# moss-lab/ScanFold

Hardware: NVIDIA B200
Metric: windows/sec (MFE+100 shuffles+ED) (higher is better)
Workload: dtype int32

## Files before the change

include/scanfold_b200.h:

```cpp
#ifndef SCANFOLD_B200_H
#define SCANFOLD_B200_H
#include <stdint.h>
#ifdef __cplusplus
extern "C" {
#endif
#if defined(__GNUC__)
#pragma GCC visibility push(default)
#endif

#define SFB_VERSION 100
#define SFB_INF 10000000

#define SFB_E_ARG (-1)
#define SFB_E_PARAMS (-2)
#define SFB_E_CUDA (-3)
#define SFB_E_STATE (-4)
#define SFB_E_RANGE (-5)

#define SFB_SHUFFLE_MONO 0
#define SFB_SHUFFLE_DI 1

typedef struct sfb_model {
    double temperature;
    int32_t max_bp_span;
// ... 69 lines not shown
int sfb_accumulate_export(sfb_partner_table *table, int row0, int n_rows, int32_t *d_count, int32_t *d_first_seen,
                          int64_t *d_sums);
int sfb_accumulate_merge(sfb_partner_table *table, int row0, int n_rows, const int32_t *d_count,
                         const int32_t *d_first_seen, const int64_t *d_sums);
int sfb_accumulate_compact(sfb_partner_table *table, int row0, int n_rows, int64_t *n_entries);
int sfb_accumulate_fetch(sfb_partner_table *table, int32_t *nparts, int32_t *partner, int32_t *count,
                         int32_t *first_seen, int64_t *sums);
int sfb_accumulate_launches(const sfb_partner_table *table);
void sfb_accumulate_free(sfb_partner_table *table);

typedef struct sfb_pairprob_table sfb_pairprob_table;
int sfb_pairprob_begin(int32_t L, int32_t W, int32_t step, int32_t first_window, int32_t n_windows,
                       sfb_pairprob_table **table);
int sfb_scan_plan_pairprob(sfb_scan_plan *plan, sfb_pairprob_table *table);
int sfb_pairprob_export(sfb_pairprob_table *table, int row0, int n_rows, int64_t *d_rows);
int sfb_pairprob_merge(sfb_pairprob_table *table, int row0, int n_rows, const int64_t *d_rows);
int sfb_pairprob_compact(sfb_pairprob_table *table, int row0, int n_rows, double cutoff, int64_t *n_pairs);
int sfb_pairprob_fetch(sfb_pairprob_table *table, double *paired, int32_t *i, int32_t *j, double *p);
void sfb_pairprob_free(sfb_pairprob_table *table);

#define SFB_MICROBENCH_ADDMIN 0
#define SFB_MICROBENCH_SMEM_LD32 1
#define SFB_MICROBENCH_DFMA 2
int sfb_microbench(int which, double *ops_per_s);

#if defined(__GNUC__)
#pragma GCC visibility pop
#endif
#ifdef __cplusplus
}
#endif
#endif
```

scanfold_b200/csrc/mfe3.cu:

```cuda
#include <cstddef>
#include <cstdio>
#include <cstdlib>
#include <type_traits>

#include "device_common.cuh"

namespace sfb {
namespace {

constexpr int INF16 = 16000;
constexpr int TABLE_ENV16 = 2000;
constexpr int FIN16 = 4000;
constexpr int LOW16 = -12000;
constexpr int R32 = 32;
constexpr int R16 = 16;
constexpr int SEG = 25;

struct alignas(16) Tab3 {
    short stack[64], mmI[200], mm1n[200], mm23[200], mmH[200];
    short mlclose[200];
    short mlstem[8 * 36];
    short ext[8 * 36];
    short tAU[8];
    short bulge1;
// ... 14 lines not shown
bool g_mfe3_ok = false;

constexpr int BIG = 1 << 20;


__device__ __forceinline__ int lds_s16(unsigned a) {
    int v;
    asm volatile("ld.shared.s16 %0, [%1];" : "=r"(v) : "r"(a));
    return v;
}
__device__ __forceinline__ unsigned lds_u32(unsigned a) {
    unsigned v;
    asm volatile("ld.shared.u32 %0, [%1];" : "=r"(v) : "r"(a));
    return v;
}
__device__ __forceinline__ int4 lds_v4(unsigned a) {
    int4 v;
    asm volatile("ld.shared.v4.s32 {%0, %1, %2, %3}, [%4];" : "=r"(v.x), "=r"(v.y), "=r"(v.z), "=r"(v.w) : "r"(a));
    return v;
}
__device__ __forceinline__ void sts_u16(unsigned a, int v) {
    asm volatile("st.shared.u16 [%0], %1;" ::"r"(a), "h"((short)v));
}

template <int P, bool FMG = false>
struct Smem3 {
    static constexpr int KSM = FMG ? 4 : 2;
    static constexpr int PR = P <= 64 ? P + 2 : ((P + 2 + 63) / 64) * 64 - 2;
    static constexpr int PRW = (P + 3) | 1;
    Tab3 tb;
    short ne[R32 * PR], no[R32 * PR], m8[R32 * PR];
    unsigned rpa[R32 * PRW];
    unsigned rpq[R32 * PRW];
    short g[R16 * PR];
    short rc[R16 * PR];
    short fm[FMG ? 8 : P * P];
    short decp[KSM * 8 * PR];
    short partc[4 * PR], parts[4 * PR];
    short f5[P + 8];
    static constexpr int LP = P;
    alignas(16) int list[(4 * LP + 16) * 4];
    unsigned char ctx[R16 * PR];
    unsigned char sx[P + 8];
    unsigned char sx5[P + 8], sx3[P + 8];
    alignas(16) int cnt[4];
    int wq[2];
    short scp[P + 8];
    int minv[32];
    int fbest[32];
    alignas(8) int stepinfo[(P / 2 + 4) * 2];
};

__host__ __device__ __forceinline__ int tri4(int d, int W) {
    return (d - 4) * W - ((d - 1) * d / 2 - 6);
}

__host__ __device__ __forceinline__ int ksplit(int D, int W, bool fmg = false) {
    if (fmg) return D >= 71 ? 4 : (D >= 36 ? 2 : 1);
    return (D < 36 || (W - 1 - D) / 2 + 1 <= 16) ? 1 : 2;
}

__device__ int hairpin_special3(const MfeTables *T, const Tab3 &tb, const unsigned char *sx, int i, int j, int type) {
    const int u = j - i - 1;
    int e = T->hairpin_len[u];
    auto key = [&](int n) {
        int k = 0, mul = 1;
        for (int t = 0; t < n; t++) {
            k += sx[i + 1 + t] * mul;
            mul *= 5;
        }
        return k;
    };
    if (u == 4) {
// ... 20 lines not shown
    if (nl == 0) return T->stack[type][t2];
    if (ns == 0) {
        int e = T->bulge[nl];
        if (nl == 1)
            e += T->stack[type][t2];
        else
            e += (type > 2 ? au : 0) + (t2 > 2 ? au : 0);
        return e;
    }
    if (ns == 1) {
        if (nl == 1) return T->int11[type][t2][si1][sj1];
        if (nl == 2) return n1 == 1 ? T->int21[type][t2][si1][sq1][sj1] : T->int21[t2][type][sq1][si1][sp1];
        return T->internal_loop[nl + 1] + min(T->max_ninio, (nl - ns) * T->ninio) + T->mismatch1nI[type][si1][sj1] +
               T->mismatch1nI[t2][sq1][sp1];
    }
    if (ns == 2) {
        if (nl == 2) return T->int22[type][t2][si1][sp1][sq1][sj1];
        if (nl == 3) return T->internal_loop[5] + T->ninio + T->mismatch23I[type][si1][sj1] + T->mismatch23I[t2][sq1][sp1];
    }
    return T->internal_loop[nl + ns] + min(T->max_ninio, (nl - ns) * T->ninio) + T->mismatchI[type][si1][sj1] +
           T->mismatchI[t2][sq1][sp1];
}

template <int P, bool FMG, class SMT>
__device__ bool traceback3(SMT &sm, const short *fm, const MfeTables *T, const short *cx, short *pt, int W, int lane) {
    const Tab3 &tb = sm.tb;
    const unsigned char *sx = sm.sx;
    const unsigned full = 0xffffffffu;
    static_assert(sizeof(sm.list) >= 3 * (P + 8) * sizeof(int), "the traceback stack lives in the list area");
    int *stk = reinterpret_cast<int *>(sm.list);
    auto ptype = [&](int a, int b) { return (int)tb.ptype[sx[a + 1] * 6 + sx[b + 1]]; };
    auto CC = [&](int i, int j) {
        const int v = cx[tri4(j - i, W) + i];
        return v >= FIN16 ? INF : v - tb.ext[ptype(i, j) * 36 + sx[i] * 6 + sx[j + 2]];
    };
    auto MM = [&](int i, int j) {
        if (j - i <= TURN) return INF;
        int v;
        if constexpr (FMG) v = __ldcg(fm + i * P + j);
        else v = fm[i * P + j];
        return v >= FIN16 ? INF : v;
    };
    for (int k = lane; k < W; k += 32) pt[k] = 0;
    int sp = 1;
    if (lane == 0) {
        stk[0] = 0;
        stk[1] = W - 1;
        stk[2] = 0;
    }
    __syncwarp();
    while (sp > 0) {
        sp--;
        int i = stk[3 * sp], j = stk[3 * sp + 1];
        const int ml = stk[3 * sp + 2];
        __syncwarp();
        bool have_pair = false;
        if (j < i + TURN + 1) continue;
        const int fij = ml ? MM(i, j) : (int)sm.f5[j + 1];
        const int mij1 = MM(i, j - 1);
        const int fi = ml ? (mij1 < INF ? mij1 + tb.MLbase : INF) : (int)sm.f5[j];
        auto push = [&](int a, int b, int c) {
            if (lane == 0) {
// ... 87 lines not shown
            if (traced) continue;
            const int en = cij - tb.mlclose[(tb.rtype[type] * 5 + sx[j]) * 5 + sx[i + 2]];
            int kf = -1;
            for (int k0 = i + 2 + TURN; k0 < j - 2 - TURN && kf < 0; k0 += 32) {
                const int k = k0 + lane;
                bool hit = false;
                if (k < j - 2 - TURN) {
                    const int a = MM(i + 1, k), b = MM(k + 1, j - 1);
                    hit = a < INF && b < INF && en == a + b;
                }
                const unsigned m = __ballot_sync(full, hit);
                if (m) kf = k0 + __ffs(m) - 1;
            }
            if (kf < 0) return false;
            push(i + 1, kf, 1);
            push(kf + 1, j - 1, 1);
            break;
        }
        __syncwarp();
    }
    return true;
}

template <int P, int NW, int OCC, bool FMG>
__global__ void __launch_bounds__(NW * 32, OCC)
mfe3_kernel(MfeLaunch L, const MfeTables *__restrict__ T, const Tab3 *__restrict__ gtab) {
    extern __shared__ __align__(16) unsigned char smem_raw[];
    using SM = Smem3<P, FMG>;
    SM &sm = *reinterpret_cast<SM *>(smem_raw);
    constexpr int NT = NW * 32, PR = SM::PR;
    const int tid = threadIdx.x, warp = tid >> 5, lane = tid & 31;
    const unsigned full = 0xffffffffu;
    {
        const int *src = reinterpret_cast<const int *>(gtab);
        int *dst = reinterpret_cast<int *>(&sm.tb);
        static_assert(sizeof(Tab3) % 4 == 0, "Tab3 is copied as 32-bit words");
        for (int k = tid; k < (int)(sizeof(Tab3) / 4); k += NT) dst[k] = src[k];
    }
    const Tab3 &tb = sm.tb;
    const unsigned char *sx = sm.sx;
    const int W = L.W;
    constexpr int LP = SM::LP;
    const int npairs = (W - TURN) / 2 + 1;
    for (int st = tid; st < npairs; st += NT) {
        const int d0 = TURN + 2 + 2 * st;
        const int nseg0 = d0 < W ? (W - d0 + SEG - 1) / SEG : 0, nseg1 = d0 + 1 < W ? (W - d0 - 1 + SEG - 1) / SEG : 0;
        const int nF = d0 - 2 < W ? (W - (d0 - 2) + 30) / 31 : 0;
        const int D = d0 + 1;
        const int ntile = D <= W - 1 ? (W - 1 - D) / 2 + 1 : 0;
        const int KS = ksplit(D, W, FMG), ksh = KS == 4 ? 2 : KS >> 1 ;
        const int kwsh = ntile > 16 ? 0 : (ntile > 8 ? 1 : 2), TPW = 32 >> kwsh;
        const int nT = ((ntile + TPW - 1) >> (5 - kwsh)) << ksh;
        reinterpret_cast<int2 *>(sm.stepinfo)[st] =
            make_int2(nseg0 | ((nseg0 + nseg1) << 8) | (nF << 16), ntile | (ksh << 8) | (kwsh << 12) | (nT << 16));
    }
    short *gC = reinterpret_cast<short *>(L.gscratch) + (size_t)blockIdx.x * L.gscratch_per_cta;
    auto ldfm = [&](const short *q) -> short {
        if constexpr (FMG) return __ldcg(q);
        else return *q;
    };
// ... 18 lines not shown
    const int UC = U < 12 ? U + 12 : (U > MAXLOOP ? MAXLOOP : U);
    const int UB10 = U < 11 ? 11 : (U > MAXLOOP ? MAXLOOP : U), UB18 = U < 20 ? 20 : (U > MAXLOOP ? MAXLOOP : U);
    const int UB26 = U < 28 ? 28 : (U > MAXLOOP ? MAXLOOP : U);
    const int kA = ((UA & 1) ? O_NO : O_NE) + 3 + (UA >> 1), kC = O_M8 + UC - 1;
    const int g6a = c3_sG6[0], g6b = c3_sG6[1], g6c = c3_sG6[2], g9 = c3_cap[9], g10 = c3_cap[10];

    auto build_list = [&](int d) {
        const int ncells = W - d, slot = d & 3;
        constexpr int NCH = (P + 31) / 32;
        int tt[NCH];
#pragma unroll
        for (int k = 0; k < NCH; k++) {
            const int i = k * 32 + lane;
            tt[k] = i < ncells ? tb.ptype[sm.sx5[i + 1] * 6 + sm.sx3[i + d + 1]] : 0;
        }
        int nl = 0;
#pragma unroll
        for (int k = 0; k < NCH; k++) {
            if (k * 32 < ncells) {
                const int i = k * 32 + lane, t = tt[k];
                const unsigned m = __ballot_sync(full, t != 0);
                if (t) {
                    const int mi = (t * 5 + sx[i + 2]) * 5 + sx[i + d];
                    const int4 en = make_int4(i, tb.mmI[mi], tb.mm1n[mi], tb.tAU[t]);
                    reinterpret_cast<int4 *>(sm.list)[slot * LP + nl + __popc(m & ((1u << lane) - 1))] = en;
                }
                nl += __popc(m);
            }
        }
        if (lane == 0) sm.cnt[slot] = nl;
    };
    auto decof = [&](int d, int xi) {
        if (d < 2 * TURN + 3) return INF16;
        const int Dsrc = (d & 1) ? ((xi & 1) ? d + 1 : d - 1) : d;
        const int ks = ksplit(Dsrc, W, FMG);
        int v = sm.decp[(d & 7) * PR + xi];
        for (int kp = 1; kp < ks; kp++) v = min(v, (int)sm.decp[(kp * 8 + (d & 7)) * PR + xi]);
        return v;
    };
    auto unit_P = [&](int d, int c) {
        const int slot = d & 3, n = sm.cnt[slot];
        const int idx = c * 32 + lane;
        const bool active = idx < n;
        const int i = active ? sm.list[(slot * LP + idx) * 4] : 0;
        const int j = i + d;
        const int type = tb.ptype[sx[i + 1] * 6 + sx[j + 1]];
        const int si1 = sx[i + 2], sj1 = sx[j];
        const int mi = (type * 5 + si1) * 5 + sj1;
        int aT = INF16;
        auto inner = [&](int u1, int u2, int &cc, int &t2, int &sp1, int &sq1) {
            const int dd = d - 2 - u1 - u2, p = i + 1 + u1, q = j - 1 - u2;
            const bool ok = dd > TURN;
            cc = ok ? sm.rc[(dd & (R16 - 1)) * PR + p] : INF16;
            t2 = ok ? sm.ctx[(dd & (R16 - 1)) * PR + p] : 0;
            sp1 = sx[p];
            sq1 = sx[q + 2];
        };
        int cc, t2, sp1, sq1;
        {
            inner(1, 1, cc, t2, sp1, sq1);
            aT = min(aT, cc + __ldg(&T->int11[type][t2][si1][sj1]));
            int eh = __ldg(&T->hairpin_len[d - 1]) + tb.mmH[mi];
            if (d <= 7 && active) eh = hairpin_special3(T, tb, sx, i, j, type);
            aT = min(aT, eh);
            inner(1, 2, cc, t2, sp1, sq1);
            aT = min(aT, cc + __ldg(&T->int21[type][t2][si1][sq1][sj1]));
            inner(2, 1, cc, t2, sp1, sq1);
            aT = min(aT, cc + __ldg(&T->int21[t2][type][sq1][si1][sp1]));
            inner(2, 2, cc, t2, sp1, sq1);
            aT = min(aT, cc + __ldg(&T->int22[type][t2][si1][sp1][sq1][sj1]));
            inner(2, 3, cc, t2, sp1, sq1);
            aT = min(aT, cc + tb.il5_ninio + tb.mm23[mi] + tb.mm23[(t2 * 5 + sq1) * 5 + sp1]);
            inner(3, 2, cc, t2, sp1, sq1);
            aT = min(aT, cc + tb.il5_ninio + tb.mm23[mi] + tb.mm23[(t2 * 5 + sq1) * 5 + sp1]);
            auto grow = [&](int dd, int p) { return dd > TURN ? (int)sm.g[(dd & (R16 - 1)) * PR + p] : INF16; };
            int aG = min(grow(d - 8, i + 3) + g6a, min(grow(d - 8, i + 4) + g6b, grow(d - 8, i + 5) + g6c));
            aG = min(aG, min(grow(d - 11, i + 3), grow(d - 11, i + 8)) + g9);
            aG = min(aG, min(grow(d - 12, i + 3), grow(d - 12, i + 9)) + g10);
            aT = min(aT, aG + tb.mmI[mi]);
        }
        if (active) sm.parts[slot * PR + i] = (short)min(aT, INF16);
    };

    int minv = 0;

    auto unit_S = [&](int d, int sg) {
        const int ncells = W - d;
        const int x = sg * SEG - 7 + lane;
        const bool valid = x >= 0 && x < ncells;
        const int i = valid ? x : 0, j = i + d;
        const int c5 = sm.sx5[i + 1], c3 = sm.sx3[j + 1];
        const int pc = sm.partc[(d & 3) * PR + i], ps = sm.parts[(d & 3) * PR + i];
        const int o2 = ((d - 2) & (R16 - 1)) * PR + i + 1, o3 = ((d - 3) & (R16 - 1)) * PR + i + 1;
        const int rc2 = sm.rc[o2], cx2 = sm.ctx[o2];
        const int rc3a = sm.rc[o3], cx3a = sm.ctx[o3], rc3b = sm.rc[o3 + 1], cx3b = sm.ctx[o3 + 1];
        const int dm = decof(d - 2, i + 1);
        const int si0 = sx[i], si2 = sx[i + 2], sj0 = sx[j], sj2 = sx[j + 2];
        int scs = 0;
        if (L.sc) scs = sm.scp[i] + sm.scp[j - 1];
        const int t = valid ? tb.ptype[c5 * 6 + c3] : 0;
        const int t2 = tb.rtype[t];
        const int st2 = tb.stack[t * 8 + cx2], st3a = tb.stack[t * 8 + cx3a], st3b = tb.stack[t * 8 + cx3b];
        const int mlc = tb.mlclose[(t2 * 5 + sj0) * 5 + si2];
        const int m2 = (t2 * 5 + sj2) * 5 + si0;
        const int xI = tb.mmI[m2], x1n = tb.mm1n[m2], xAU = tb.tAU[t2];
        int e = min(pc, ps);
        if (d - 2 > TURN) e = min(e, rc2 + st2 + scs);
        if (d - 3 > TURN) e = min(e, min(rc3a + st3a, rc3b + st3b) + tb.bulge1);
        e = min(e, dm + mlc);
        if (!t || e >= FIN16) e = INF16;
        int vg = INF16, v1 = INF16, vb = INF16;
        if (t && i > 0 && j < W - 1 && e < FIN16) {
            vg = e + xI;
            v1 = e + x1n;
            vb = e + xAU;
        }
        const int g1 = __shfl_up_sync(full, vg, 1), g2 = __shfl_up_sync(full, vg, 2);
        const int g3 = __shfl_up_sync(full, vg, 3), g4 = __shfl_up_sync(full, vg, 4);
        const int ne = min(g2, min(min(g1, g3) + tb.w2, min(vg, g4) + tb.w4));
        const int no = min(min(g1, g2) + tb.w1, min(vg, g3) + tb.w3);
        int m8 = min(vg, g1);
        m8 = min(m8, __shfl_up_sync(full, m8, 2));
        m8 = min(m8, __shfl_up_sync(full, m8, 4));
        if (valid && lane >= 7) {
            minv = min(minv, e);
            const int o16 = (d & (R16 - 1)) * PR + i, o32 = (d & (R32 - 1)) * PR + i;
            sm.rc[o16] = (short)e;
            sm.ctx[o16] = (unsigned char)t2;
            sm.g[o16] = (short)vg;
            {
                short *wa = reinterpret_cast<short *>(sm.rpa) + 2 * ((d & (R32 - 1)) * PRW + i);
                short *wq = reinterpret_cast<short *>(sm.rpq) + 2 * ((d & (R32 - 1)) * PRW + j);
                wa[0] = (short)vb;
                if (i > 0) wa[-1] = (short)v1;
                wq[0] = (short)vb;
                wq[3] = (short)v1;
            }
            sm.ne[o32] = (short)ne;
            sm.no[o32] = (short)no;
            sm.m8[o32] = (short)m8;
            gC[tri4(d, W) + i] = (short)(e < FIN16 ? e + tb.ext[t * 36 + sx[i] * 6 + sx[j + 2]] : INF16);
        }
    };

    auto unit_F = [&](int dA, int u) {
        const int nc0 = dA > TURN ? W - dA : 0, nc1 = dA + 1 < W ? W - dA - 1 : 0;
        const int x = u * 31 + lane;
        const bool v0 = x < nc0;
        const int xx = v0 ? x : max(nc0 - 1, 0);
        auto stemof = [&](int d, int xi) {
            const int o16 = (d & (R16 - 1)) * PR + xi;
            const int e = sm.rc[o16];
            const int t = tb.rtype[sm.ctx[o16]];
            return e < FIN16 ? e + tb.mlstem[t * 36 + sx[xi] * 6 + sx[xi + d + 2]] : INF16;
        };
        const int x1c = min(x, max(nc1 - 1, 0));
        const int s0 = min(decof(dA, xx), stemof(dA, xx));
        const int s1 = min(decof(dA + 1, x1c), stemof(dA + 1, x1c));
        int m0 = INF16;
        if (nc0 > 0) {
            m0 = s0;
            if (dA - 1 > TURN)
                m0 = min(m0, min((int)ldfm(fm + (xx + 1) * P + xx + dA), (int)ldfm(fm + xx * P + xx + dA - 1)) + tb.MLbase);
            if (m0 >= FIN16) m0 = INF16;
            if (v0) {
                minv = min(minv, m0);
                fm[x * P + x + dA] = (short)m0;
                fm[(x + dA) * P + x] = (short)m0;
            }
        }
        const int m0n = __shfl_down_sync(full, m0, 1);
        if (lane < 31 && x < nc1) {
            const int d = dA + 1;
            int m1 = min(s1, min(m0, m0n) + tb.MLbase);
// ... 61 lines not shown
                const unsigned a = pa[0], b = pb[0];
                acc0 = __viaddmin_s16x2(a, __byte_perm(b, 0, 0x1010), acc0);
                acc1 = __viaddmin_s16x2(a, __byte_perm(b, 0, 0x3232), acc1);
            }
        }
        if (kwsh >= 1) {
            acc0 = __vmins2(acc0, __shfl_xor_sync(full, acc0, 16));
            acc1 = __vmins2(acc1, __shfl_xor_sync(full, acc1, 16));
        }
        if (kwsh == 2) {
            acc0 = __vmins2(acc0, __shfl_xor_sync(full, acc0, 8));
            acc1 = __vmins2(acc1, __shfl_xor_sync(full, acc1, 8));
        }
        if (valid && kq == 0) {
            auto fin = [](int v) { return (short)(v >= FIN16 ? INF16 : v); };
            short *dp = sm.decp + kp * 8 * PR;
            dp[(D & 7) * PR + i] = fin((short)(acc0 & 0xffffu));
            dp[((D - 1) & 7) * PR + i + 1] = fin((int)acc0 >> 16);
            if (j + 1 < W) {
                dp[((D + 1) & 7) * PR + i] = fin((short)(acc1 & 0xffffu));
                dp[(D & 7) * PR + i + 1] = fin((int)acc1 >> 16);
            }
        }
    };

    for (int fold = blockIdx.x; fold < L.n_fold; fold += gridDim.x) {
        __syncthreads();
        for (int k = tid; k < W + 2; k += NT) {
            const bool edge = k == 0 || k == W + 1;
            const int code = edge ? 5 : L.seqs[(size_t)fold * W + k - 1];
            const char ch = (L.hc && !edge) ? (char)L.hc[(size_t)fold * W + k - 1] : '.';
            sm.sx[k] = (unsigned char)code;
            sm.sx5[k] = (unsigned char)((ch == 'x' || ch == '>') ? 5 : code);
            sm.sx3[k] = (unsigned char)((ch == 'x' || ch == '<') ? 5 : code);
        }
        {
            const int4 inf4 = make_int4(INF16 * 65537, INF16 * 65537, INF16 * 65537, INF16 * 65537);
            int4 *p = reinterpret_cast<int4 *>(sm.ne);
            constexpr int n16 = (int)((offsetof(SM, decp) - offsetof(SM, ne) + 15) / 16);
            for (int k = tid; k < n16; k += NT) p[k] = inf4;
            for (int k = tid; k < 4 * PR; k += NT) sm.partc[k] = INF16;
            if constexpr (FMG) {
                int4 *q = reinterpret_cast<int4 *>(fm);
                for (int k = tid; k < P * P / 8; k += NT) q[k] = inf4;
            }
        }
// ... 88 lines not shown
                int my = draw();
                while (my < total) {
                    const int nx = draw();
                    if (my < uP) {
                        unit_T(d0 + 1, my, ntile, ksh, kwsh);
                    } else if (my < uS) {
                        const int it = my - uP;
                        unit_P(it < nch2 ? d0 + 2 : d0 + 3, it < nch2 ? it : it - nch2);
                    } else if (my < uL) {
                        const int u = my - uS;
                        unit_S(u >= nseg0 ? d0 + 1 : d0, u >= nseg0 ? u - nseg0 : u);
                    } else if (my < uF) {
                        build_list(d0 + 4 + (my - uL));
                    } else if (my < uC) {
                        unit_F(d0 - 2, my - uF);
                    } else {
                        const int ci = my - uC, ds = ci >= nc2;
                        const int c = (ds ? ci - nc2 : ci) * CH;
                        unit_C(d0 + 2 + ds, c, min(c + CH, ds ? n3 : n2));
                    }
                    my = nx;
                }
            } else {
                const int uP = nS, uT = uP + nP, uF = uT + nT, uL = uF + nF, nH = uL + 2;
                for (int u = warp; u < nH; u += NW) {
                    if (u < uP) {
                        unit_S(u >= nseg0 ? d0 + 1 : d0, u >= nseg0 ? u - nseg0 : u);
                    } else if (u < uT) {
                        const int it = u - uP;
                        unit_P(it < nch2 ? d0 + 2 : d0 + 3, it < nch2 ? it : it - nch2);
                    } else if (u < uF) {
                        unit_T(d0 + 1, u - uT, ntile, ksh, kwsh);
                    } else if (u < uL) {
                        unit_F(d0 - 2, u - uF);
                    } else {
                        build_list(d0 + 4 + (u - uL));
                    }
                }
                int c = warp - nH % NW;
                if (c < 0) c += NW;
#pragma unroll 1
                for (int ds = 0; ds < 2; ds++) {
                    const int d = d0 + 2 + ds, n = ds ? n3 : n2;
                    if (c < n) {
                        const int slot = (d - 2 - UB) & (R32 - 1);
                        const unsigned sb = (unsigned)__cvta_generic_to_shared(smb);
                        const unsigned aA = sb + 2 * (kA + ((d - 2 - UA) & (R32 - 1)) * PR);
                        const unsigned aB10 = sb + 2 * (O_M8 + 10 + ((d - 2 - UB10) & (R32 - 1)) * PR);
                        const unsigned aB18 = sb + 2 * (O_M8 + 18 + ((d - 2 - UB18) & (R32 - 1)) * PR);
                        const unsigned aB26 = sb + 2 * (O_M8 + 26 + ((d - 2 - UB26) & (R32 - 1)) * PR);
                        const unsigned aC = sb + 2 * (kC + ((d - 2 - UC) & (R32 - 1)) * PR);
                        const unsigned aR = (unsigned)__cvta_generic_to_shared(sm.rpa + slot * PRW + 1);
                        const unsigned aL = (unsigned)__cvta_generic_to_shared(sm.rpq + slot * PRW + d - 1);
                        const unsigned aP = (unsigned)__cvta_generic_to_shared(sm.partc + (d & 3) * PR);
                        unsigned aLst = (unsigned)__cvta_generic_to_shared(reinterpret_cast<const int4 *>(sm.list) + (d & 3) * LP + c);
                        int4 en = lds_v4(aLst);
                        for (; c < n; c += NW) {
                            const int i = en.x, eI = en.y, e1 = en.z, eB = en.w;
                            aLst += NW * 16;
                            en = lds_v4(aLst);
                            const unsigned i2 = 2 * i, i4 = 4 * i;
                            const unsigned wr = lds_u32(aR + i4), wl = lds_u32(aL + i4);
                            const int xa = lds_s16(aA + i2), xb10 = lds_s16(aB10 + i2), xb18 = lds_s16(aB18 + i2);
                            const int xb26 = lds_s16(aB26 + i2), xc = lds_s16(aC + i2);
                            const unsigned wm = __vmins2(wr, wl);
                            const int xb = (int)(short)(wm & 0xffffu), x1 = (int)wm >> 16;
                            int g = xa + cA;
                            g = __viaddmin_s32(xb10, cB10, g);
                            int g2 = xb18 + cB18;
                            g2 = __viaddmin_s32(xb26, cB26, g2);
                            g = __viaddmin_s32(xc, cC, g);
                            const int aB = xb + cSB, a1 = x1 + cS1;
                            int v = min(g, g2) + eI;
                            v = __viaddmin_s32(a1, e1, v);
                            v = __viaddmin_s32(aB, eB, v);
                            v = __reduce_min_sync(full, v);
                            if (lane == 0) sts_u16(aP + i2, v);
                        }
                    }
                    c -= n;
                }
            }
            __syncthreads();
        }

        {
            short *cx = sm.ne;
            const int ntri = tri4(W, W);
            for (int k = tid; k < ntri; k += NT) cx[k] = __ldcg(gC + k);
            for (int k = tid; k <= min(W, TURN + 1); k += NT) sm.f5[k] = 0;
            const int minw = __reduce_min_sync(full, minv);
            if (lane == 0) sm.minv[warp] = minw;
            __syncthreads();
            constexpr int LPR = 8, NPART = NW > LPR ? NW / LPR : 1;
            for (int len0 = TURN + 2; len0 <= W; len0 += LPR) {
                for (int t = warp % LPR; t < LPR; t += NW) {
                    const int len = len0 + t, j = len - 1, part = warp / LPR;
                    int best = INF16;
                    if (len <= W && part < NPART)
                        for (int i = lane + 32 * part; i <= min(j - TURN - 1, len0 - 1); i += 32 * NPART)
                            best = min(best, sm.f5[i] + cx[tri4(j - i, W) + i]);
                    best = __reduce_min_sync(full, best);
                    if (lane == 0 && part < NPART) sm.fbest[t + LPR * part] = best;
                }
                __syncthreads();
                if (tid == 0) {
// ... 2 lines not shown
#pragma unroll
                    for (int t = 0; t < LPR; t++) {
                        if (len0 + t <= W) {
#pragma unroll
                            for (int h = 0; h < NPART; h++) run = min(run, sm.fbest[t + LPR * h]);
#pragma unroll
                            for (int q = 0; q + 5 <= t; q++) {
                                const int i = len0 + q, j = len0 + t - 1;
                                run = min(run, f[q] + cx[tri4(j - i, W) + i]);
                            }
                            f[t] = run;
                            sm.f5[len0 + t] = (short)run;
                        }
                    }
                }
                __syncthreads();
            }
            int mv = sm.minv[0];
            for (int q = 1; q < NW; q++) mv = min(mv, sm.minv[q]);
            if (tid == 0) L.e_out[fold] = mv < LOW16 ? MFE_REDO : (int)sm.f5[W];
            if (L.pair_tbl && mv >= LOW16) {
                short *pt = sm.partc;
                if (warp == 0) {
                    const bool ok = traceback3<P, FMG>(sm, fm, T, cx, pt, W, lane);
                    if (!ok && lane == 0) L.e_out[fold] = MFE_REDO;
                }
                __syncthreads();
                for (int k = tid; k < W; k += NT) L.pair_tbl[(size_t)fold * W + k] = pt[k];
            }
        }
    }
}

template <int P, int NW, int OCC, bool FMG = false>
void launch_mfe3_t(const MfeLaunch &L, const MfeTables *d_tab, int n_sm, cudaStream_t stream) {
    const size_t smem = sizeof(Smem3<P, FMG>);
    static bool cfg = false;
    if (!cfg) {
        cudaFuncSetAttribute(mfe3_kernel<P, NW, OCC, FMG>, cudaFuncAttributeMaxDynamicSharedMemorySize, (int)smem);
        cfg = true;
    }
    const int grid = L.n_fold < n_sm * OCC ? L.n_fold : n_sm * OCC;
    mfe3_kernel<P, NW, OCC, FMG><<<grid, NW * 32, smem, stream>>>(L, d_tab, g_dtab3);
}

}

static_assert(sizeof(Smem3<200>) <= 227 * 1024, "the 200-nt configuration must fit one SM");
static_assert(sizeof(Smem3<300, true>) <= 227 * 1024, "the 300-nt configuration must fit one SM");
static_assert(300 * 300 % 8 == 0, "the global matrix is cleared with 16-byte stores");
bool mfe3_supports(int W) { return g_mfe3_ok && W >= 16 && W <= 300; }

size_t mfe3_scratch_shorts_per_cta(int W) {
    const size_t tri = ((size_t)tri4(W, W) + 63) & ~(size_t)63;
    return tri + (W > 200 ? (size_t)300 * 300 : 0);
}

int mfe3_max_ctas(int n_sm, int W) { return n_sm * (W <= 64 ? 4 : (W <= 120 ? 2 : 1)); }

void mfe3_upload_tables(const MfeTables &M) {
    static Tab3 h;
    bool fit = true;
    auto s16 = [&fit](int v) {
        fit = fit && v >= -TABLE_ENV16 && v <= TABLE_ENV16;
        return (short)v;
    };
    auto mm = [](int t, int a, int b) { return (t * 5 + a) * 5 + b; };
    static const int rt[8] = {0, 2, 1, 4, 3, 6, 5, 7};
    for (int a = 0; a < 8; a++)
        for (int b = 0; b < 8; b++) h.stack[a * 8 + b] = s16(M.stack[a][b]);
    for (int t = 0; t < 8; t++) {
        h.tAU[t] = s16(t > 2 ? M.TerminalAU : 0);
        h.rtype[t] = (unsigned char)rt[t];
        for (int a = 0; a < 5; a++)
            for (int b = 0; b < 5; b++) {
                h.mmI[mm(t, a, b)] = s16(M.mismatchI[t][a][b]);
                h.mm1n[mm(t, a, b)] = s16(M.mismatch1nI[t][a][b]);
                h.mm23[mm(t, a, b)] = s16(M.mismatch23I[t][a][b]);
                h.mmH[mm(t, a, b)] = s16(M.mismatchH[t][a][b]);
                h.mlclose[mm(t, a, b)] = s16(M.mismatchM[t][a][b] + (t > 2 ? M.TerminalAU : 0) + M.MLintern + M.MLclosing);
            }
// ... 29 lines not shown
    for (int u = 0; u < 32; u++) {
        const bool ok = u <= MAXLOOP && M.internal_loop[u < 31 ? u : 30] < INF;
        sI[u] = ok ? M.internal_loop[u] : INF16;
        sC[u] = ok ? M.internal_loop[u] + M.max_ninio : INF16;
        s1[u] = ok ? M.internal_loop[u] + std::min(M.max_ninio, (u - 2) * M.ninio) : INF16;
        sB[u] = (u <= MAXLOOP && M.bulge[u < 31 ? u : 30] < INF) ? M.bulge[u] : INF16;
    }
    for (int k = 0; k < 3; k++) {
        const int u1 = 2 + k, u2 = 6 - u1, diff = u1 > u2 ? u1 - u2 : u2 - u1;
        s6[k] = M.internal_loop[6] < INF ? M.internal_loop[6] + std::min(M.max_ninio, diff * M.ninio) : INF16;
    }
    s6[3] = INF16;
    cudaMemcpyToSymbol(c3_il, sI, sizeof(sI));
    cudaMemcpyToSymbol(c3_cap, sC, sizeof(sC));
    cudaMemcpyToSymbol(c3_size1, s1, sizeof(s1));
    cudaMemcpyToSymbol(c3_sizeB, sB, sizeof(sB));
    cudaMemcpyToSymbol(c3_sG6, s6, sizeof(s6));
    if (!g_dtab3) cudaMalloc(&g_dtab3, sizeof(Tab3));
    cudaMemcpy(g_dtab3, &h, sizeof(Tab3), cudaMemcpyHostToDevice);
}

void launch_mfe3(const MfeLaunch &L, const MfeTables *d_tab, int n_sm, cudaStream_t stream, int *n_launches) {
    if (L.n_fold <= 0) return;
    static const int nw = getenv("SFB_MFE3_WARPS") ? atoi(getenv("SFB_MFE3_WARPS")) : 12;
    if (L.W <= 64)
        launch_mfe3_t<64, 4, 4>(L, d_tab, n_sm, stream);
    else if (L.W > 200)
        launch_mfe3_t<300, 16, 1, true>(L, d_tab, n_sm, stream);
    else if (L.W > 120)
        launch_mfe3_t<200, 16, 1>(L, d_tab, n_sm, stream);
    else if (nw == 4)
        launch_mfe3_t<120, 4, 2>(L, d_tab, n_sm, stream);
    else if (nw == 12)
        launch_mfe3_t<120, 12, 2>(L, d_tab, n_sm, stream);
    else if (nw == 16)
        launch_mfe3_t<120, 16, 2>(L, d_tab, n_sm, stream);
    else
        launch_mfe3_t<120, 8, 2>(L, d_tab, n_sm, stream);
    if (n_launches) (*n_launches)++;
}

}
```

scanfold_b200/csrc/microbench.cu:

```cuda
#include <cuda_runtime.h>

#include "../../include/scanfold_b200.h"

namespace {

constexpr int MB_THREADS = 1024;
constexpr int MB_CHAINS = 8;

__global__ void __launch_bounds__(MB_THREADS) addmin_kernel(int *out, int iters, int x) {
    int acc[MB_CHAINS];
#pragma unroll
    for (int k = 0; k < MB_CHAINS; k++) acc[k] = threadIdx.x * (k + 1) + blockIdx.x;
    for (int it = 0; it < iters; it++) {
#pragma unroll
        for (int rep = 0; rep < 4; rep++) {
#pragma unroll
            for (int k = 0; k < MB_CHAINS; k++) acc[k] = __viaddmin_s32(acc[k], x, acc[(k + 1) % MB_CHAINS]);
        }
    }
    int s = 0;
#pragma unroll
    for (int k = 0; k < MB_CHAINS; k++) s ^= acc[k];
    if (s == 0x7fffffff) out[0] = s;
}
// ... 16 lines not shown
    }
    int s = a0 ^ a1 ^ a2 ^ a3;
    if (s == 0x7fffffff) out[0] = s;
}

__global__ void __launch_bounds__(MB_THREADS) dfma_kernel(int *out, int iters, double x) {
    double acc[MB_CHAINS];
#pragma unroll
    for (int k = 0; k < MB_CHAINS; k++) acc[k] = 1e-3 * (threadIdx.x + k) + blockIdx.x;
    const double y = 1.0 - 1e-9 * x;
    for (int it = 0; it < iters; it++) {
#pragma unroll
        for (int rep = 0; rep < 4; rep++) {
#pragma unroll
            for (int k = 0; k < MB_CHAINS; k++) acc[k] = fma(acc[k], y, x);
        }
    }
    double s = 0.;
#pragma unroll
    for (int k = 0; k < MB_CHAINS; k++) s += acc[k];
    if (s == 12345.678) out[0] = 1;
}

}

extern "C" int sfb_microbench(int which, double *ops_per_s) {
    if (!ops_per_s || (which != SFB_MICROBENCH_ADDMIN && which != SFB_MICROBENCH_SMEM_LD32 && which != SFB_MICROBENCH_DFMA)) return SFB_E_ARG;
    int dev = 0, n_sm = 0;
    if (cudaGetDevice(&dev) != cudaSuccess) return SFB_E_CUDA;
    cudaDeviceGetAttribute(&n_sm, cudaDevAttrMultiProcessorCount, dev);
    int *d_out = nullptr;
    if (cudaMalloc(&d_out, 64) != cudaSuccess) return SFB_E_CUDA;
    cudaEvent_t e0, e1;
    cudaEventCreate(&e0);
    cudaEventCreate(&e1);
    const int grid = n_sm * 2;
    const int iters = which == SFB_MICROBENCH_ADDMIN ? 8192 : (which == SFB_MICROBENCH_DFMA ? 1024 : 2048);
    double best = 0.;
    for (int rep = 0; rep < 4; rep++) {
        cudaEventRecord(e0);
        if (which == SFB_MICROBENCH_ADDMIN)
            addmin_kernel<<<grid, MB_THREADS>>>(d_out, iters, rep + 1);
        else if (which == SFB_MICROBENCH_DFMA)
            dfma_kernel<<<grid, MB_THREADS>>>(d_out, iters, 1e-3 * (rep + 1));
        else
            smem_kernel<<<grid, MB_THREADS>>>(d_out, iters);
        cudaEventRecord(e1);
        if (cudaEventSynchronize(e1) != cudaSuccess) break;
        float ms = 0.f;
// ... 13 lines not shown
```

Baseline: 16750.

## Add tensor-memory MFE kernel variant for 120-nt windows at three CTAs per SM

Adds a TM variant of the 120-nt MFE kernel. It keeps the multiloop column values in Blackwell tensor memory (tcgen05 alloc/ld/st) and stores the FM matrix as a packed triangle. The multiloop decomposition now runs as a paired 16-bit viaddmin over TMEM columns and triangle rows. The variant also packs list entries into 8 bytes, drops the rpq mirror array and shrinks the rc/ctx ring, so shared memory fits three CTAs per SM instead of two. It becomes the default path for W in 65..120 (8 warps, occupancy 3), at the cost of TMEM load latency and extra fences. The diff also adds TMEM and LDS latency microbenchmarks.

```diff
diff --git a/include/scanfold_b200.h b/include/scanfold_b200.h
--- a/include/scanfold_b200.h
+++ b/include/scanfold_b200.h
@@ -115,6 +115,8 @@
 #define SFB_MICROBENCH_ADDMIN 0
 #define SFB_MICROBENCH_SMEM_LD32 1
 #define SFB_MICROBENCH_DFMA 2
+#define SFB_MICROBENCH_TMEM_LD_LATENCY 3
+#define SFB_MICROBENCH_LDS_LATENCY 4
 int sfb_microbench(int which, double *ops_per_s);
 
 #if defined(__GNUC__)
diff --git a/scanfold_b200/csrc/mfe3.cu b/scanfold_b200/csrc/mfe3.cu
--- a/scanfold_b200/csrc/mfe3.cu
+++ b/scanfold_b200/csrc/mfe3.cu
@@ -60,25 +60,53 @@
 __device__ __forceinline__ void sts_u16(unsigned a, int v) {
     asm volatile("st.shared.u16 [%0], %1;" ::"r"(a), "h"((short)v));
 }
-
-template <int P, bool FMG = false>
+__device__ __forceinline__ int2 lds_v2(unsigned a) {
+    int2 v;
+    asm volatile("ld.shared.v2.s32 {%0, %1}, [%2];" : "=r"(v.x), "=r"(v.y) : "r"(a));
+    return v;
+}
+
+__device__ __forceinline__ void tmem_ld16(unsigned ta, unsigned (&r)[16]) {
+    asm volatile(
+        "tcgen05.ld.sync.aligned.32x32b.x16.b32 {%0, %1, %2, %3, %4, %5, %6, %7, %8, %9, %10, %11, %12, %13, %14, %15}, [%16];"
+        : "=r"(r[0]), "=r"(r[1]), "=r"(r[2]), "=r"(r[3]), "=r"(r[4]), "=r"(r[5]), "=r"(r[6]), "=r"(r[7]), "=r"(r[8]),
+          "=r"(r[9]), "=r"(r[10]), "=r"(r[11]), "=r"(r[12]), "=r"(r[13]), "=r"(r[14]), "=r"(r[15])
+        : "r"(ta));
+    asm volatile("tcgen05.wait::ld.sync.aligned;"
+                 : "+r"(r[0]), "+r"(r[1]), "+r"(r[2]), "+r"(r[3]), "+r"(r[4]), "+r"(r[5]), "+r"(r[6]), "+r"(r[7]), "+r"(r[8]),
+                   "+r"(r[9]), "+r"(r[10]), "+r"(r[11]), "+r"(r[12]), "+r"(r[13]), "+r"(r[14]), "+r"(r[15])::"memory");
+}
+__device__ __forceinline__ void tmem_st1(unsigned ta, unsigned v) {
+    asm volatile("tcgen05.st.sync.aligned.32x32b.x1.b32 [%0], {%1};" ::"r"(ta), "r"(v) : "memory");
+}
+__device__ __forceinline__ void tmem_fence_before_sync() { asm volatile("tcgen05.fence::before_thread_sync;" ::: "memory"); }
+__device__ __forceinline__ void tmem_fence_after_sync() { asm volatile("tcgen05.fence::after_thread_sync;" ::: "memory"); }
+
+__host__ __device__ constexpr int fm3_row(int b) {
+    return (b & 1) ? 2 * ((b >> 1) - 1) * ((b >> 1) - 1) + 2 * (b >> 1) - 3 : 2 * ((b >> 1) - 1) * ((b >> 1) - 1) - 2;
+}
+constexpr int TM_COLS = 64;
+
+template <int P, bool FMG = false, bool TM = false>
 struct Smem3 {
-    static constexpr int KSM = FMG ? 4 : 2;
+    static constexpr int KSM = FMG ? 4 : (TM ? 1 : 2);
+    static constexpr int RC = TM ? 8 : R16;
+    static constexpr int LW = TM ? 2 : 4;
     static constexpr int PR = P <= 64 ? P + 2 : ((P + 2 + 63) / 64) * 64 - 2;
     static constexpr int PRW = (P + 3) | 1;
     Tab3 tb;
     short ne[R32 * PR], no[R32 * PR], m8[R32 * PR];
     unsigned rpa[R32 * PRW];
-    unsigned rpq[R32 * PRW];
+    unsigned rpq[TM ? 1 : R32 * PRW];
     short g[R16 * PR];
-    short rc[R16 * PR];
-    short fm[FMG ? 8 : P * P];
+    short rc[RC * PR];
+    short fm[FMG ? 8 : (TM ? fm3_row(P) : P * P)];
     short decp[KSM * 8 * PR];
     short partc[4 * PR], parts[4 * PR];
     short f5[P + 8];
     static constexpr int LP = P;
-    alignas(16) int list[(4 * LP + 16) * 4];
-    unsigned char ctx[R16 * PR];
+    alignas(16) int list[(4 * LP + 16) * LW];
+    unsigned char ctx[RC * PR];
     unsigned char sx[P + 8];
     unsigned char sx5[P + 8], sx3[P + 8];
     alignas(16) int cnt[4];
@@ -87,6 +115,7 @@
     int minv[32];
     int fbest[32];
     alignas(8) int stepinfo[(P / 2 + 4) * 2];
+    unsigned taddr;
 };
 
 __host__ __device__ __forceinline__ int tri4(int d, int W) {
@@ -153,7 +182,7 @@
            T->mismatchI[t2][sq1][sp1];
 }
 
-template <int P, bool FMG, class SMT>
+template <int P, bool FMG, bool TM, class SMT>
 __device__ bool traceback3(SMT &sm, const short *fm, const MfeTables *T, const short *cx, short *pt, int W, int lane) {
     const Tab3 &tb = sm.tb;
     const unsigned char *sx = sm.sx;
@@ -169,6 +198,7 @@
         if (j - i <= TURN) return INF;
         int v;
         if constexpr (FMG) v = __ldcg(fm + i * P + j);
+        else if constexpr (TM) v = fm[fm3_row(j) + i];
         else v = fm[i * P + j];
         return v >= FIN16 ? INF : v;
     };
@@ -302,11 +332,13 @@
     return true;
 }
 
-template <int P, int NW, int OCC, bool FMG>
+template <int P, int NW, int OCC, bool FMG, bool TM = false>
 __global__ void __launch_bounds__(NW * 32, OCC)
 mfe3_kernel(MfeLaunch L, const MfeTables *__restrict__ T, const Tab3 *__restrict__ gtab) {
     extern __shared__ __align__(16) unsigned char smem_raw[];
-    using SM = Smem3<P, FMG>;
+    using SM = Smem3<P, FMG, TM>;
+    static_assert(!TM || (NW % 4 == 0 && !FMG), "TM: units are dealt to warps by lane quarter (warp % 4)");
+    constexpr int RCM = SM::RC - 1;
     SM &sm = *reinterpret_cast<SM *>(smem_raw);
     constexpr int NT = NW * 32, PR = SM::PR;
     const int tid = threadIdx.x, warp = tid >> 5, lane = tid & 31;
@@ -316,6 +348,17 @@
         int *dst = reinterpret_cast<int *>(&sm.tb);
         static_assert(sizeof(Tab3) % 4 == 0, "Tab3 is copied as 32-bit words");
         for (int k = tid; k < (int)(sizeof(Tab3) / 4); k += NT) dst[k] = src[k];
+    }
+    if constexpr (TM) {
+        if (warp == 0) {
+            asm volatile("tcgen05.alloc.cta_group::1.sync.aligned.shared::cta.b32 [%0], %1;" ::"r"(
+                             (unsigned)__cvta_generic_to_shared(&sm.taddr)),
+                         "n"(TM_COLS));
+            asm volatile("tcgen05.relinquish_alloc_permit.cta_group::1.sync.aligned;");
+        }
+        tmem_fence_before_sync();
+        __syncthreads();
+        tmem_fence_after_sync();
     }
     const Tab3 &tb = sm.tb;
     const unsigned char *sx = sm.sx;
@@ -380,8 +423,12 @@
                 const unsigned m = __ballot_sync(full, t != 0);
                 if (t) {
                     const int mi = (t * 5 + sx[i + 2]) * 5 + sx[i + d];
-                    const int4 en = make_int4(i, tb.mmI[mi], tb.mm1n[mi], tb.tAU[t]);
-                    reinterpret_cast<int4 *>(sm.list)[slot * LP + nl + __popc(m & ((1u << lane) - 1))] = en;
+                    const int e = slot * LP + nl + __popc(m & ((1u << lane) - 1));
+                    if constexpr (TM)
+                        reinterpret_cast<int2 *>(sm.list)[e] = make_int2(i | ((int)tb.mmI[mi] << 16),
+                                                                         ((int)tb.mm1n[mi] & 0xffff) | ((int)tb.tAU[t] << 16));
+                    else
+                        reinterpret_cast<int4 *>(sm.list)[e] = make_int4(i, tb.mmI[mi], tb.mm1n[mi], tb.tAU[t]);
                 }
                 nl += __popc(m);
             }
@@ -390,6 +437,7 @@
     };
     auto decof = [&](int d, int xi) {
         if (d < 2 * TURN + 3) return INF16;
+        if constexpr (TM) return (int)sm.decp[(d & 7) * PR + xi];
         const int Dsrc = (d & 1) ? ((xi & 1) ? d + 1 : d - 1) : d;
         const int ks = ksplit(Dsrc, W, FMG);
         int v = sm.decp[(d & 7) * PR + xi];
@@ -400,7 +448,7 @@
         const int slot = d & 3, n = sm.cnt[slot];
         const int idx = c * 32 + lane;
         const bool active = idx < n;
-        const int i = active ? sm.list[(slot * LP + idx) * 4] : 0;
+        const int i = active ? sm.list[(slot * LP + idx) * SM::LW] & 0xffff : 0;
         const int j = i + d;
         const int type = tb.ptype[sx[i + 1] * 6 + sx[j + 1]];
         const int si1 = sx[i + 2], sj1 = sx[j];
@@ -409,8 +457,8 @@
         auto inner = [&](int u1, int u2, int &cc, int &t2, int &sp1, int &sq1) {
             const int dd = d - 2 - u1 - u2, p = i + 1 + u1, q = j - 1 - u2;
             const bool ok = dd > TURN;
-            cc = ok ? sm.rc[(dd & (R16 - 1)) * PR + p] : INF16;
-            t2 = ok ? sm.ctx[(dd & (R16 - 1)) * PR + p] : 0;
+            cc = ok ? sm.rc[(dd & RCM) * PR + p] : INF16;
+            t2 = ok ? sm.ctx[(dd & RCM) * PR + p] : 0;
             sp1 = sx[p];
             sq1 = sx[q + 2];
         };
@@ -449,7 +497,7 @@
         const int i = valid ? x : 0, j = i + d;
         const int c5 = sm.sx5[i + 1], c3 = sm.sx3[j + 1];
         const int pc = sm.partc[(d & 3) * PR + i], ps = sm.parts[(d & 3) * PR + i];
-        const int o2 = ((d - 2) & (R16 - 1)) * PR + i + 1, o3 = ((d - 3) & (R16 - 1)) * PR + i + 1;
+        const int o2 = ((d - 2) & RCM) * PR + i + 1, o3 = ((d - 3) & RCM) * PR + i + 1;
         const int rc2 = sm.rc[o2], cx2 = sm.ctx[o2];
         const int rc3a = sm.rc[o3], cx3a = sm.ctx[o3], rc3b = sm.rc[o3 + 1], cx3b = sm.ctx[o3 + 1];
         const int dm = decof(d - 2, i + 1);
@@ -482,17 +530,19 @@
         m8 = min(m8, __shfl_up_sync(full, m8, 4));
         if (valid && lane >= 7) {
             minv = min(minv, e);
-            const int o16 = (d & (R16 - 1)) * PR + i, o32 = (d & (R32 - 1)) * PR + i;
-            sm.rc[o16] = (short)e;
-            sm.ctx[o16] = (unsigned char)t2;
+            const int o16 = (d & (R16 - 1)) * PR + i, o32 = (d & (R32 - 1)) * PR + i, orc = (d & RCM) * PR + i;
+            sm.rc[orc] = (short)e;
+            sm.ctx[orc] = (unsigned char)t2;
             sm.g[o16] = (short)vg;
             {
                 short *wa = reinterpret_cast<short *>(sm.rpa) + 2 * ((d & (R32 - 1)) * PRW + i);
                 short *wq = reinterpret_cast<short *>(sm.rpq) + 2 * ((d & (R32 - 1)) * PRW + j);
                 wa[0] = (short)vb;
                 if (i > 0) wa[-1] = (short)v1;
-                wq[0] = (short)vb;
-                wq[3] = (short)v1;
+                if constexpr (!TM) {
+                    wq[0] = (short)vb;
+                    wq[3] = (short)v1;
+                }
             }
             sm.ne[o32] = (short)ne;
             sm.no[o32] = (short)no;
@@ -507,7 +557,7 @@
         const bool v0 = x < nc0;
         const int xx = v0 ? x : max(nc0 - 1, 0);
         auto stemof = [&](int d, int xi) {
-            const int o16 = (d & (R16 - 1)) * PR + xi;
+            const int o16 = (d & RCM) * PR + xi;
             const int e = sm.rc[o16];
             const int t = tb.rtype[sm.ctx[o16]];
             return e < FIN16 ? e + tb.mlstem[t * 36 + sx[xi] * 6 + sx[xi + d + 2]] : INF16;
@@ -615,6 +665,77 @@
                 dp[(D & 7) * PR + i + 1] = fin((int)acc1 >> 16);
             }
         }
+    };
+
+    auto unit_F3 = [&](int dA, int q) {
+        const int nc0 = dA > TURN ? W - dA : 0, nc1 = dA + 1 < W ? W - dA - 1 : 0;
+        if (32 * q >= max(nc0, nc1)) return;
+        const int x = 32 * q + lane;
+        auto stemof = [&](int d, int xi) {
+            const int o = (d & RCM) * PR + xi;
+            const int e = sm.rc[o];
+            const int t = tb.rtype[sm.ctx[o]];
+            return e < FIN16 ? e + tb.mlstem[t * 36 + sx[xi] * 6 + sx[xi + d + 2]] : INF16;
+        };
+        auto m0of = [&](int y) {
+            int m = min(decof(dA, y), stemof(dA, y));
+            if (dA - 1 > TURN) m = min(m, min((int)fm[fm3_row(y + dA) + y + 1], (int)fm[fm3_row(y + dA - 1) + y]) + tb.MLbase);
+            return m >= FIN16 ? INF16 : m;
+        };
+        int m0 = INF16, m0n = INF16, m1 = INF16;
+        if (nc0 > 0) {
+            const int last = nc0 - 1;
+            const int a = m0of(min(x, last)), b = m0of(min(x + 1, last));
+            m0 = x < nc0 ? a : INF16;
+            m0n = x + 1 < nc0 ? b : INF16;
+        }
+        if (x < nc1) {
+            const int s1 = min(decof(dA + 1, x), stemof(dA + 1, x));
+            m1 = min(s1, min(m0, m0n) + tb.MLbase);
+            if (m1 >= FIN16) m1 = INF16;
+            minv = min(minv, m1);
+            fm[fm3_row(x + dA + 1) + x] = (short)m1;
+        }
+        if (x < nc0) {
+            minv = min(minv, m0);
+            fm[fm3_row(x + dA) + x] = (short)m0;
+        }
+        tmem_st1(sm.taddr + ((unsigned)(32 * q) << 16) + ((dA - TURN) >> 1), ((unsigned)m0 & 0xffffu) | ((unsigned)m1 << 16));
+    };
+
+    auto unit_T3 = [&](int d, int q) {
+        const int ncell = W - d;
+        if (d < 2 * TURN + 3 || 32 * q >= ncell) return;
+        const int x = 32 * q + lane;
+        const int i = min(x, ncell - 1), j = i + d;
+        const int C = (d - 8) >> 1;
+        const unsigned ta = sm.taddr + ((unsigned)(32 * q) << 16);
+        const unsigned rowb = (unsigned)__cvta_generic_to_shared(fm + fm3_row(j) + i + 4);
+        unsigned acc = INF16 * 65537u;
+        if ((d & 1) == 0) {
+            for (int c0 = 0; c0 <= C; c0 += 16) {
+                unsigned r[16];
+                tmem_ld16(ta + c0, r);
+#pragma unroll
+                for (int z = 0; z < 16; z++)
+                    if (c0 + z <= C) acc = __viaddmin_s16x2(r[z], lds_u32(rowb + 4 * (c0 + z)), acc);
+            }
+        } else {
+            unsigned prev = lds_u32(rowb - 2);
+            for (int c0 = 0; c0 <= C; c0 += 16) {
+                unsigned r[16];
+                tmem_ld16(ta + c0, r);
+#pragma unroll
+                for (int z = 0; z < 16; z++)
+                    if (c0 + z <= C) {
+                        const unsigned nx = lds_u32(rowb + 2 + 4 * (c0 + z));
+                        acc = __viaddmin_s16x2(r[z], __byte_perm(prev, nx, 0x5432), acc);
+                        prev = nx;
+                    }
+            }
+        }
+        const int v = min((int)(short)(acc & 0xffffu), (int)acc >> 16);
+        if (x < ncell) sm.decp[(d & 7) * PR + i] = (short)(v >= FIN16 ? INF16 : v);
     };
 
     for (int fold = blockIdx.x; fold < L.n_fold; fold += gridDim.x) {
@@ -749,7 +870,7 @@
                     my = nx;
                 }
             } else {
-                const int uP = nS, uT = uP + nP, uF = uT + nT, uL = uF + nF, nH = uL + 2;
+                const int uP = nS, uT = uP + nP, uF = uT + (TM ? 8 : nT), uL = uF + (TM ? 4 : nF), nH = uL + 2;
                 for (int u = warp; u < nH; u += NW) {
                     if (u < uP) {
                         unit_S(u >= nseg0 ? d0 + 1 : d0, u >= nseg0 ? u - nseg0 : u);
@@ -757,9 +878,11 @@
                         const int it = u - uP;
                         unit_P(it < nch2 ? d0 + 2 : d0 + 3, it < nch2 ? it : it - nch2);
                     } else if (u < uF) {
-                        unit_T(d0 + 1, u - uT, ntile, ksh, kwsh);
+                        if constexpr (TM) unit_T3(d0 + 1 + ((u - uT) >> 2), warp & 3);
+                        else unit_T(d0 + 1, u - uT, ntile, ksh, kwsh);
                     } else if (u < uL) {
-                        unit_F(d0 - 2, u - uF);
+                        if constexpr (TM) unit_F3(d0 - 2, warp & 3);
+                        else unit_F(d0 - 2, u - uF);
                     } else {
                         build_list(d0 + 4 + (u - uL));
                     }
@@ -778,16 +901,43 @@
                         const unsigned aB26 = sb + 2 * (O_M8 + 26 + ((d - 2 - UB26) & (R32 - 1)) * PR);
                         const unsigned aC = sb + 2 * (kC + ((d - 2 - UC) & (R32 - 1)) * PR);
                         const unsigned aR = (unsigned)__cvta_generic_to_shared(sm.rpa + slot * PRW + 1);
-                        const unsigned aL = (unsigned)__cvta_generic_to_shared(sm.rpq + slot * PRW + d - 1);
+                        const unsigned aL = TM ? (unsigned)__cvta_generic_to_shared(sm.rpa + slot * PRW + UB + 1)
+                                               : (unsigned)__cvta_generic_to_shared(sm.rpq + slot * PRW + d - 1);
                         const unsigned aP = (unsigned)__cvta_generic_to_shared(sm.partc + (d & 3) * PR);
-                        unsigned aLst = (unsigned)__cvta_generic_to_shared(reinterpret_cast<const int4 *>(sm.list) + (d & 3) * LP + c);
-                        int4 en = lds_v4(aLst);
+                        constexpr int LB = SM::LW * 4;
+                        unsigned aLst = (unsigned)__cvta_generic_to_shared(sm.list) + ((d & 3) * LP + c) * LB;
+                        int4 en;
+                        if constexpr (TM) {
+                            const int2 e2 = lds_v2(aLst);
+                            en = make_int4(e2.x, e2.y, 0, 0);
+                        } else {
+                            en = lds_v4(aLst);
+                        }
                         for (; c < n; c += NW) {
-                            const int i = en.x, eI = en.y, e1 = en.z, eB = en.w;
-                            aLst += NW * 16;
-                            en = lds_v4(aLst);
+                            int i, eI, e1, eB;
+                            if constexpr (TM) {
+                                i = en.x & 0xffff;
+                                eI = en.x >> 16;
+                                e1 = (int)(short)(en.y & 0xffff);
+                                eB = en.y >> 16;
+                            } else {
+                                i = en.x;
+                                eI = en.y;
+                                e1 = en.z;
+                                eB = en.w;
+                            }
+                            aLst += NW * LB;
+                            if constexpr (TM) {
+                                const int2 e2 = lds_v2(aLst);
+                                en = make_int4(e2.x, e2.y, 0, 0);
+                            } else {
+                                en = lds_v4(aLst);
+                            }
                             const unsigned i2 = 2 * i, i4 = 4 * i;
-                            const unsigned wr = lds_u32(aR + i4), wl = lds_u32(aL + i4);
+                            const unsigned wr = lds_u32(aR + i4);
+                            unsigned wl;
+                            if constexpr (TM) wl = __byte_perm(lds_u32(aL + i4), lds_u32(aL - 8 + i4), 0x7610);
+                            else wl = lds_u32(aL + i4);
                             const int xa = lds_s16(aA + i2), xb10 = lds_s16(aB10 + i2), xb18 = lds_s16(aB18 + i2);
                             const int xb26 = lds_s16(aB26 + i2), xc = lds_s16(aC + i2);
                             const unsigned wm = __vmins2(wr, wl);
@@ -808,7 +958,12 @@
                     c -= n;
                 }
             }
+            if constexpr (TM) {
+                asm volatile("tcgen05.wait::st.sync.aligned;" ::: "memory");
+                tmem_fence_before_sync();
+            }
             __syncthreads();
+            if constexpr (TM) tmem_fence_after_sync();
         }
 
         {
@@ -857,7 +1012,7 @@
             if (L.pair_tbl && mv >= LOW16) {
                 short *pt = sm.partc;
                 if (warp == 0) {
-                    const bool ok = traceback3<P, FMG>(sm, fm, T, cx, pt, W, lane);
+                    const bool ok = traceback3<P, FMG, TM>(sm, fm, T, cx, pt, W, lane);
                     if (!ok && lane == 0) L.e_out[fold] = MFE_REDO;
                 }
                 __syncthreads();
@@ -865,18 +1020,24 @@
             }
         }
     }
-}
-
-template <int P, int NW, int OCC, bool FMG = false>
+    if constexpr (TM) {
+        tmem_fence_before_sync();
+        __syncthreads();
+        tmem_fence_after_sync();
+        if (warp == 0) asm volatile("tcgen05.dealloc.cta_group::1.sync.aligned.b32 %0, %1;" ::"r"(sm.taddr), "n"(TM_COLS));
+    }
+}
+
+template <int P, int NW, int OCC, bool FMG = false, bool TM = false>
 void launch_mfe3_t(const MfeLaunch &L, const MfeTables *d_tab, int n_sm, cudaStream_t stream) {
-    const size_t smem = sizeof(Smem3<P, FMG>);
+    const size_t smem = sizeof(Smem3<P, FMG, TM>);
     static bool cfg = false;
     if (!cfg) {
-        cudaFuncSetAttribute(mfe3_kernel<P, NW, OCC, FMG>, cudaFuncAttributeMaxDynamicSharedMemorySize, (int)smem);
+        cudaFuncSetAttribute(mfe3_kernel<P, NW, OCC, FMG, TM>, cudaFuncAttributeMaxDynamicSharedMemorySize, (int)smem);
         cfg = true;
     }
     const int grid = L.n_fold < n_sm * OCC ? L.n_fold : n_sm * OCC;
-    mfe3_kernel<P, NW, OCC, FMG><<<grid, NW * 32, smem, stream>>>(L, d_tab, g_dtab3);
+    mfe3_kernel<P, NW, OCC, FMG, TM><<<grid, NW * 32, smem, stream>>>(L, d_tab, g_dtab3);
 }
 
 }
@@ -884,6 +1045,8 @@
 static_assert(sizeof(Smem3<200>) <= 227 * 1024, "the 200-nt configuration must fit one SM");
 static_assert(sizeof(Smem3<300, true>) <= 227 * 1024, "the 300-nt configuration must fit one SM");
 static_assert(300 * 300 % 8 == 0, "the global matrix is cleared with 16-byte stores");
+static_assert(sizeof(Smem3<120, false, true>) <= 75 * 1024, "the 120-nt tensor-memory configuration must fit three CTAs per SM");
+static_assert(3 * TM_COLS <= 512 && (120 - 1 - TURN) / 2 < TM_COLS, "three CTAs' FML columns fit tensor memory");
 bool mfe3_supports(int W) { return g_mfe3_ok && W >= 16 && W <= 300; }
 
 size_t mfe3_scratch_shorts_per_cta(int W) {
@@ -891,7 +1054,7 @@
     return tri + (W > 200 ? (size_t)300 * 300 : 0);
 }
 
-int mfe3_max_ctas(int n_sm, int W) { return n_sm * (W <= 64 ? 4 : (W <= 120 ? 2 : 1)); }
+int mfe3_max_ctas(int n_sm, int W) { return n_sm * (W <= 64 ? 4 : (W <= 120 ? 3 : 1)); }
 
 void mfe3_upload_tables(const MfeTables &M) {
     static Tab3 h;
@@ -967,13 +1130,15 @@
 
 void launch_mfe3(const MfeLaunch &L, const MfeTables *d_tab, int n_sm, cudaStream_t stream, int *n_launches) {
     if (L.n_fold <= 0) return;
-    static const int nw = getenv("SFB_MFE3_WARPS") ? atoi(getenv("SFB_MFE3_WARPS")) : 12;
+    static const int nw = getenv("SFB_MFE3_WARPS") ? atoi(getenv("SFB_MFE3_WARPS")) : 0;
     if (L.W <= 64)
         launch_mfe3_t<64, 4, 4>(L, d_tab, n_sm, stream);
     else if (L.W > 200)
         launch_mfe3_t<300, 16, 1, true>(L, d_tab, n_sm, stream);
     else if (L.W > 120)
         launch_mfe3_t<200, 16, 1>(L, d_tab, n_sm, stream);
+    else if (nw == 0)
+        launch_mfe3_t<120, 8, 3, false, true>(L, d_tab, n_sm, stream);
     else if (nw == 4)
         launch_mfe3_t<120, 4, 2>(L, d_tab, n_sm, stream);
     else if (nw == 12)
diff --git a/scanfold_b200/csrc/microbench.cu b/scanfold_b200/csrc/microbench.cu
--- a/scanfold_b200/csrc/microbench.cu
+++ b/scanfold_b200/csrc/microbench.cu
@@ -62,9 +62,85 @@
     if (s == 12345.678) out[0] = 1;
 }
 
+constexpr int LAT_ITERS = 4096;
+
+__device__ __forceinline__ unsigned tmem_ld_x16_first(unsigned taddr, unsigned &last) {
+    unsigned r[16];
+    asm volatile(
+        "tcgen05.ld.sync.aligned.32x32b.x16.b32 {%0, %1, %2, %3, %4, %5, %6, %7, %8, %9, %10, %11, %12, %13, %14, %15}, [%16];"
+        : "=r"(r[0]), "=r"(r[1]), "=r"(r[2]), "=r"(r[3]), "=r"(r[4]), "=r"(r[5]), "=r"(r[6]), "=r"(r[7]), "=r"(r[8]),
+          "=r"(r[9]), "=r"(r[10]), "=r"(r[11]), "=r"(r[12]), "=r"(r[13]), "=r"(r[14]), "=r"(r[15])
+        : "r"(taddr));
+    asm volatile("tcgen05.wait::ld.sync.aligned;" : "+r"(r[0]), "+r"(r[15])::"memory");
+    last = r[15];
+    return r[0];
+}
+
+__global__ void __launch_bounds__(128) tmem_latency_kernel(long long *out) {
+    __shared__ unsigned taddr_s;
+    const int warp = threadIdx.x >> 5;
+    if (warp == 0) {
+        asm volatile("tcgen05.alloc.cta_group::1.sync.aligned.shared::cta.b32 [%0], 32;" ::"r"(
+            (unsigned)__cvta_generic_to_shared(&taddr_s)));
+        asm volatile("tcgen05.relinquish_alloc_permit.cta_group::1.sync.aligned;");
+    }
+    asm volatile("tcgen05.fence::before_thread_sync;");
+    __syncthreads();
+    asm volatile("tcgen05.fence::after_thread_sync;");
+    const unsigned tbase = taddr_s;
+    const unsigned quarter = tbase + ((unsigned)(32 * warp) << 16);
+    for (int c = 0; c < 32; c++) asm volatile("tcgen05.st.sync.aligned.32x32b.x1.b32 [%0], {%1};" ::"r"(quarter + c), "r"(0));
+    asm volatile("tcgen05.wait::st.sync.aligned;" ::: "memory");
+    unsigned v = 0, last = 0;
+    const long long t0 = clock64();
+    for (int it = 0; it < LAT_ITERS; it++) v = tmem_ld_x16_first(quarter + (v & 15), last) | (last & 1);
+    const long long t1 = clock64();
+    if (threadIdx.x == 0) out[0] = t1 - t0;
+    if (v == 12345) out[1] = v;
+    asm volatile("tcgen05.fence::before_thread_sync;");
+    __syncthreads();
+    asm volatile("tcgen05.fence::after_thread_sync;");
+    if (warp == 0) asm volatile("tcgen05.dealloc.cta_group::1.sync.aligned.b32 %0, 32;" ::"r"(tbase));
+}
+
+__global__ void __launch_bounds__(128) lds_latency_kernel(long long *out) {
+    __shared__ int buf[1024];
+    for (int k = threadIdx.x; k < 1024; k += 128) buf[k] = 0;
+    __syncthreads();
+    const unsigned base = (unsigned)__cvta_generic_to_shared(buf) + 4 * (threadIdx.x & 31);
+    unsigned v = 0;
+    const long long t0 = clock64();
+    for (int it = 0; it < LAT_ITERS; it++) asm volatile("ld.shared.u32 %0, [%1];" : "=r"(v) : "r"(base + (v & 15) * 128));
+    const long long t1 = clock64();
+    if (threadIdx.x == 0) out[0] = t1 - t0;
+    if (v == 12345) out[1] = v;
+}
+
+int latency_cycles(int which, double *cycles) {
+    long long *d_out = nullptr;
+    if (cudaMalloc(&d_out, 16) != cudaSuccess) return SFB_E_CUDA;
+    double best = 0.;
+    for (int rep = 0; rep < 4; rep++) {
+        if (which == SFB_MICROBENCH_TMEM_LD_LATENCY)
+            tmem_latency_kernel<<<1, 128>>>(d_out);
+        else
+            lds_latency_kernel<<<1, 128>>>(d_out);
+        long long t = 0;
+        if (cudaMemcpy(&t, d_out, sizeof(t), cudaMemcpyDeviceToHost) != cudaSuccess) break;
+        const double c = (double)t / LAT_ITERS;
+        if (rep > 0 && (best == 0. || c < best)) best = c;
+    }
+    cudaFree(d_out);
+    if (cudaGetLastError() != cudaSuccess || best <= 0.) return SFB_E_CUDA;
+    *cycles = best;
+    return 0;
+}
+
 }
 
 extern "C" int sfb_microbench(int which, double *ops_per_s) {
+    if (ops_per_s && (which == SFB_MICROBENCH_TMEM_LD_LATENCY || which == SFB_MICROBENCH_LDS_LATENCY))
+        return latency_cycles(which, ops_per_s);
     if (!ops_per_s || (which != SFB_MICROBENCH_ADDMIN && which != SFB_MICROBENCH_SMEM_LD32 && which != SFB_MICROBENCH_DFMA)) return SFB_E_ARG;
     int dev = 0, n_sm = 0;
     if (cudaGetDevice(&dev) != cudaSuccess) return SFB_E_CUDA;
```

After: 15330, median of 6. 0.915x the previous value.
